# Stanford-ILIAD/PantheonRL

Hardware: AMD Instinct MI355X
Metric: env-steps/sec (all agents) Overcooked-simple PPO self-play (higher is better)
Workload: dtype f32; 1 GPU; OvercookedMultiEnv-v0 layout=simple, PPO self-play (two independent PPO learners per GPU), synthetic (n_envs, n_steps, obs_dim) rollouts; n_envs=1024, n_steps=128, obs_dim=62, features=62, n_logits=6, batch_size=32768, n_epochs=10, agents_per_gpu=2, parallelism=2 agent(s) per gpu x1 gpu(s) = 2 learners (single process), launch_mode=graph, gemm_mode=2, action_masks=none, rollout=scripted, rollout_requested=scripted

## Files before the change

include/pantheon_hip.h:

```cpp
#ifndef PANTHEON_HIP_H
#define PANTHEON_HIP_H

#ifdef __cplusplus
extern "C" {
#endif

#define PH_ABI_VERSION 7
#define PH_HIDDEN 64
#define PH_MAX_COMP 256
#define PH_MAX_LOGITS 64
#define PH_MAX_BOX_ACT 16
#define PH_NSTAT 8
#define PH_MOD_MAX 8
#define PH_MAX_RANKS 16

#define PH_SPACE_BOX 0
#define PH_SPACE_DISCRETE 1

typedef struct ph_ctx ph_ctx;

typedef struct ph_space {
  int kind;
  int n;
  int nvec[PH_MAX_COMP];
// ... 426 lines not shown
                               float *stats_out, const ph_adap_loss *adap );
int ph_adapmult_train(ph_ctx *ctx, const ph_spec *spec, int context_size, const ph_opt_state *opt, const ph_rollout *rb,
                      const ph_ppo_hyper *hyper , int n_epochs, int batch_size, const int *perms,
                      unsigned long long perm_seed, float *stats, const ph_adap_loss *adap );

int ph_bench_ppo_grad(ph_ctx *ctx, const ph_spec *spec, const float *params, const ph_rollout *rb,
                      const ph_ppo_hyper *hyper , int batch_size, int reps, int gemm_mode,
                      float *avg_ms_out );
int ph_bench_gae(ph_ctx *ctx, const ph_rollout *rb, const float *last_values, const float *dones, double gamma,
                 double gae_lambda, int mode, int reps, float *avg_ms_out );

enum {
  PH_BENCH_WEIGHT_IMAGE = 0,
  PH_BENCH_OBS_PLANES = 1,
  PH_BENCH_ADV_STATS = 2,
  PH_BENCH_REDUCE = 3,
  PH_BENCH_REDUCE_WIDE = 4,
  PH_BENCH_ADAM = 5,
  PH_BENCH_STEP_FUSED = 6,
  PH_BENCH_BUFFER_ADD = 7,
  PH_BENCH_SLAB_FLOATS = 8,
  PH_BENCH_NKERN = 9
};
int ph_bench_train_kernels(ph_ctx *ctx, const ph_spec *spec, const ph_opt_state *scratch_opt, const ph_rollout *rb,
                           const ph_ppo_hyper *hyper , int n_epochs, int batch_size, int reps, int gemm_mode,
                           float *us_out );

int ph_feistel_indices(int n, unsigned long long perm_seed, int epoch, int start, int count, int *out );

typedef struct ph_modular {
  int num_partners;
  int n_modules;
  int module_of[PH_MOD_MAX];
  int nomain;
} ph_modular;
int ph_modular_layout(const ph_spec *spec , const ph_modular *mod , ph_layout *main_out ,
                      ph_layout *module_out , int *p_total_out );
int ph_modular_forward(ph_ctx *ctx, const ph_spec *spec, const ph_modular *mod, const float *params, int partner_idx,
                       const float *obs, int n, const unsigned char *action_mask, const float *uniforms,
                       const float *given_actions, unsigned long long seed, unsigned long long counter, int deterministic,
                       int *actions_i32, float *actions_f32, float *values, float *log_probs, float *entropy,
                       float *logits_main , float *logits_partner ,
                       const ph_rollout *rb, int pos, const float *episode_start_in, const float *pending_reward,
                       int gemm_mode);
int ph_modular_train(ph_ctx *ctx, const ph_spec *spec, const ph_modular *mod, const ph_opt_state *opt,
                     int *mod_first ,
// ... 86 lines not shown
```

pantheonrl_amd/_native.py:

```python
from __future__ import annotations

import ctypes as C
import os
from typing import Optional, Sequence

PH_HIDDEN = 64
PH_MAX_COMP = 256
PH_MAX_LOGITS = 64
PH_MAX_BOX_ACT = 16
PH_NSTAT = 8
PH_SPACE_BOX = 0
PH_SPACE_DISCRETE = 1
STAT_NAMES = ("policy_loss", "value_loss", "entropy_loss", "clip_fraction", "approx_kl", "loss", "grad_norm", "applied")

_HERE = os.path.dirname(os.path.abspath(__file__))
LIB_PATH = os.environ.get("PANTHEON_HIP_LIB") or os.path.join(_HERE, "csrc", "libpantheon_hip.so")


class NativeError(RuntimeError):
    """Raised for any non-zero status from the C ABI (message from ph_last_error)."""


class PhSpace(C.Structure):
    _fields_ = [("kind", C.c_int), ("n", C.c_int), ("nvec", C.c_int * PH_MAX_COMP)]
# ... 190 lines not shown
                ("obs_ego", C.c_void_p), ("obs_alt", C.c_void_p), ("episodes", C.c_void_p),
                ("obs_next", C.c_void_p), ("rew1", C.c_void_p), ("rew2", C.c_void_p), ("es_alt", C.c_void_p),
                ("done1", C.c_void_p), ("done2", C.c_void_p), ("running", C.c_void_p), ("can", C.c_void_p),
                ("alt_opens", C.c_void_p), ("ego_opens", C.c_void_p), ("done", C.c_void_p)]

SIGNATURES = {
    "ph_abi_version": [],
    "ph_roundrobin_env_step": [_vp, _vp, _vp, _vp, _vp, _vp, _vp, _vp, _i, _i, C.c_float, _i],
    "ph_last_error": [],
    "ph_device_count": [C.POINTER(_i)],
    "ph_ctx_create": [_i, C.POINTER(_vp)],
    "ph_ctx_destroy": [_vp],
    "ph_ctx_set_stream": [_vp, _vp],
    "ph_ctx_sync": [_vp],
    "ph_graph_begin": [_vp],
    "ph_graph_end": [_vp, C.POINTER(_i)],
    "ph_graph_launch": [_vp, _i],
    "ph_ctx_set_rng_epoch": [_vp, _vp],
    "ph_rng_epoch_advance": [_vp],
    "ph_debug_set_profile_buffer": [_vp, _vp],
    "ph_set_exclusive_device": [_vp, _i],
    "ph_ctx_step_errors": [_vp, C.POINTER(C.c_uint)],
    "ph_debug_weight_image_mismatches": [_vp, C.POINTER(PhSpec), _vp, C.POINTER(C.c_int)],
    "ph_timer_start": [_vp],
    "ph_timer_stop": [_vp, C.POINTER(C.c_float)],
    "ph_layout_of": [C.POINTER(PhSpec), C.POINTER(PhLayout)],
    "ph_debug_split_tables": [C.POINTER(PhSpec), C.POINTER(C.c_int), C.POINTER(C.c_int), C.POINTER(C.c_int)],
    "ph_debug_split_oh_tables": [C.POINTER(PhSpec), _vp, _vp, C.POINTER(_i), C.POINTER(_i), C.POINTER(_i)],
    "ph_buffer_add": [_vp, C.POINTER(PhSpec), C.POINTER(PhRollout), _i, _vp, _vp, _vp, _vp, _vp],
    "ph_buffer_add_reward": [_vp, C.POINTER(PhRollout), _i, _vp, _vp],
    "ph_buffer_add_reward_joint": [_vp, C.POINTER(PhRollout), _i, _vp, _vp, _i, _i, _vp, C.c_float],
    "ph_buffer_reset": [_vp, C.POINTER(PhSpec), C.POINTER(PhRollout)],
    "ph_gae": [_vp, C.POINTER(PhRollout), _vp, _vp, _d, _d, _i],
    "ph_policy_forward": [_vp, C.POINTER(PhSpec), _vp, _vp, _i, _vp, _vp, _vp, _ull, _ull, _i, _vp, _vp, _vp, _vp, _vp,
                          _vp, C.POINTER(PhRollout), _i, _vp, _vp, _i],
    "ph_ctx_set_joint_reward_rule": [_vp, _i],
    "ph_adapmult_layout_of": [C.POINTER(PhSpec), _i, _vp],
    "ph_adapmult_forward": [_vp, C.POINTER(PhSpec), _i, _vp, _vp, _i, _vp, _vp, _vp, _ull, _ull, _i, _vp, _vp, _vp, _vp, _vp,
                            _vp, C.POINTER(PhRollout), _i, _vp],
    "ph_adapmult_minibatch_grad": [_vp, C.POINTER(PhSpec), _i, _vp, C.POINTER(PhRollout), C.POINTER(PhPpoHyper), _vp, _i, _vp, _vp,
                                   _vp],
    "ph_adapmult_train": [_vp, C.POINTER(PhSpec), _i, C.POINTER(PhOptState), C.POINTER(PhRollout), C.POINTER(PhPpoHyper), _i, _i,
                          _vp, _ull, _vp, _vp],
    "ph_policy_act_host": [_vp, C.POINTER(PhSpec), _vp, _vp, _i, _vp, _ull, _ull, _i, _vp, _vp, _vp, C.POINTER(PhRollout), _i, _i],
    "ph_buffer_add_reward_const": [_vp, C.POINTER(PhRollout), _i, C.c_float],
    "ph_policy_step_multi": [_vp, _i, C.POINTER(PhStepCall)],
# ... 245 lines not shown
```

pantheonrl_amd/csrc/ph_abi.hip:

```cpp
#include <dlfcn.h>
#include <hip/hip_runtime.h>
#include <rccl/rccl.h>

#include <atomic>
#include <chrono>
#include <cmath>
#include <cstdio>
#include <cstdint>
#include <cstring>
#include <mutex>
#include <string>
#include <vector>

#include "ph_launch.h"
#include "ph_block.h"
#include "ph_arch.h"
#include "ph_pool.h"

namespace ph {

namespace {
struct LdsGrant {
  const void* kernel;
  int device;
// ... 81 lines not shown
  size_t slabs_cap = 0;
  float* statpart = nullptr;
  size_t statpart_cap = 0;
  float* grad = nullptr;
  size_t grad_cap = 0;
  float* blocksq = nullptr;
  size_t blocksq_cap = 0;
  float* advstats = nullptr;
  size_t advstats_cap = 0;
  float* act_stage_host = nullptr;
  float* act_stage_dev = nullptr;
  size_t act_stage_cap = 0;
  unsigned int* act_done_host = nullptr;
  unsigned int* act_done_dev = nullptr;
  unsigned int act_seq = 0;
  unsigned int* fwd_host_done = nullptr;
  int joint_reward_rule = 0;
  int wimage_zeroed_for = 0;
  size_t wimage_cap = 0;
  bool exclusive = false;
  unsigned short* wimage = nullptr;
  double* advpart = nullptr;
  size_t advpart_cap = 0;
  int* perm_idx = nullptr;
  size_t perm_idx_cap = 0;
  int* perm_phys = nullptr;
  size_t perm_phys_cap = 0;
  uint4* ximg = nullptr;
  size_t ximg_cap = 0;
  uint4* rec_pi = nullptr;
  uint4* rec_vf = nullptr;
  size_t rec_cap = 0;
  uint4* rowrec = nullptr;
  size_t rowrec_cap = 0;
  unsigned long long* step_words = nullptr;
  size_t step_words_cap = 0;
  unsigned int* step_gen = nullptr;
  float* am_buf = nullptr;
  size_t am_buf_cap = 0;
  float* adap_extra = nullptr;
  size_t adap_extra_cap = 0;
  float* adap_loss = nullptr;
  size_t adap_loss_cap = 0;
  float* scalars = nullptr;
  int* stop_flag = nullptr;
  std::vector<SpecCache> specs;
// ... 245 lines not shown
    a.prev_rew = rb->rewards + (row - rb->E);
    a.pending_reward = pending_reward;
  }
  return 0;
}

ph::AdvStatArgs adv_args_epochs(const ph_ctx* ctx, const ph_rollout* rb, const int* perms, unsigned long long perm_seed, int batch,
                                int n_mb) {
  const int N = rb->T * rb->E;
  ph::AdvStatArgs aa{};
  aa.rb_adv = rb->advantages;
  aa.T = rb->T;
  aa.E = rb->E;
  aa.perms = perms;
  aa.perm_n = (uint32_t)N;
  aa.perm_hb = ph::feistel_half_bits((uint32_t)N);
  aa.perm_seed = perm_seed;
  aa.epoch = ctx->rng_epoch;
  aa.N = N;
  aa.batch = batch;
  aa.n_mb = n_mb;
  aa.out = ctx->advstats;
  aa.partial = ctx->advpart;
  aa.idx_out = perms ? nullptr : ctx->perm_idx;
  aa.phys_out = ctx->perm_phys;
  return aa;
}
ph::AdvStatArgs adv_args_minibatch(const ph_ctx* ctx, const ph_rollout* rb, const int* indices, int nb) {
  ph::AdvStatArgs aa{};
  aa.rb_adv = rb->advantages;
  aa.T = rb->T;
  aa.E = rb->E;
  aa.perms = indices;
  aa.perm_hb = 1;
  aa.N = nb;
  aa.batch = nb;
  aa.n_mb = 1;
  aa.out = ctx->advstats;
  aa.partial = ctx->advpart;
  aa.phys_out = ctx->perm_phys;
  return aa;
}

struct MbWalk {
  int ep, start, nb;
  const int* idx;
};
MbWalk minibatch_walk(const ph_ctx* ctx, const int* perms, int N, int n_mb, int batch_size, int mbi) {
  MbWalk w;
  w.ep = mbi / n_mb;
  w.start = (mbi - w.ep * n_mb) * batch_size;
  w.nb = N - w.start < batch_size ? N - w.start : batch_size;
  w.idx = (perms ? perms : ctx->perm_idx) + (size_t)w.ep * N + w.start;
  return w;
}

ph::ReduceArgs reduce_args(const ph_ctx* ctx, const ph_ppo_hyper* hp, const ph_opt_state* opt, int P, int slab_len, const int* map,
                           int nslab, int nb, float* grad, float* stats_out) {
  ph::ReduceArgs r;
  r.slabs = ctx->slabs;
  r.nslab = nslab;
  r.nstatpart = 2 * nslab;
// ... 116 lines not shown
    return fail("hipMalloc(ctx scalars) failed");
  }
  (void)hipMemset(c->scalars, 0, 4 * sizeof(float));
  (void)hipMemset(c->stop_flag, 0, sizeof(int));
  (void)hipEventCreate(&c->ev0);
  (void)hipEventCreate(&c->ev1);
  *out = c;
  return 0;
}

int ph_ctx_destroy(ph_ctx* ctx) {
  DevGuard dev_guard(ctx);
  if (!ctx) return 0;
  (void)hipStreamSynchronize(ctx->stream);
  for (auto g : ctx->graphs)
    if (g) (void)hipGraphExecDestroy(g);
  for (auto& s : ctx->specs) {
    if (s.obs_off) (void)hipFree(s.obs_off);
    if (s.slab_map) (void)hipFree(s.slab_map);
    if (s.slab_map_split) (void)hipFree(s.slab_map_split);
    if (s.wimage_map) (void)hipFree(s.wimage_map);
    if (s.act_off) (void)hipFree(s.act_off);
  }
  void* ptrs[] = {ctx->wimage, ctx->mw.act, ctx->mw.maps, ctx->mw.kl_sum, ctx->mw.scratch, ctx->advpart, ctx->p2p_dev, ctx->slabs, ctx->statpart, ctx->grad, ctx->blocksq, ctx->advstats, ctx->perm_idx, ctx->perm_phys, ctx->ximg, ctx->rec_pi, ctx->rec_vf, ctx->rowrec, ctx->step_words, ctx->step_gen, ctx->scalars, ctx->stop_flag,
                  ctx->adap_extra, ctx->adap_loss, ctx->am_buf, ctx->pool_dev, ctx->pool_order, ctx->pool_tiles};
  for (void* p : ptrs)
    if (p) (void)hipFree(p);
  if (ctx->act_stage_host) (void)hipHostFree(ctx->act_stage_host);
  if (ctx->act_done_host) (void)hipHostFree(ctx->act_done_host);
  if (ctx->ev0) (void)hipEventDestroy(ctx->ev0);
  if (ctx->ev1) (void)hipEventDestroy(ctx->ev1);
  if (ctx->ev_grad) (void)hipEventDestroy(ctx->ev_grad);
  (void)ph_comm_destroy(ctx);
  delete ctx;
  return 0;
}

int ph_ctx_set_joint_reward_rule(ph_ctx* ctx, int rule) {
  if (!ctx) return fail("null ctx");
  if (rule != PH_JOINT_MATCH_BONUS && rule != PH_JOINT_RPS) return fail("ph_ctx_set_joint_reward_rule: unknown rule");
  ctx->joint_reward_rule = rule;
  return 0;
}

int ph_ctx_set_stream(ph_ctx* ctx, void* hip_stream) {
  DevGuard dev_guard(ctx);
  if (!ctx) return fail("null ctx");
// ... 1443 lines not shown
  }
  PH_HIP(ph::launch_obs_planes(rb->observations, (int)rows, nd.D, nd.F, ph::grad_fast_fold(nd) ? 1 : 0, ctx->ximg, rb->advantages,
                               rb->log_probs, rb->actions, rb->returns, rb->values, ctx->rowrec, ctx->stream));
  return 0;
}
void fill_adv_records(ph::AdvStatArgs& aa, const ph_ctx* ctx, const ph::NetDims& nd, const ph_rollout* rb) {
  aa.rec_pi_out = nd.split == 1 ? ctx->rec_pi : nullptr;
  aa.rec_vf_out = nd.split == 1 ? ctx->rec_vf : nullptr;
  aa.rowrec = (nd.split == 1 && rb->advantages && rb->log_probs && rb->actions && rb->returns && rb->values) ? ctx->rowrec : nullptr;
  aa.rb_logp = rb->log_probs;
  aa.rb_act = rb->actions;
  aa.rb_ret = rb->returns;
  aa.rb_val = rb->values;
}


void select_gemm(ph::NetDims& nd, int gemm_mode) {
  nd.split = (gemm_mode == 2 && nd.slab_map_split != nullptr) ? nd.split_kind : 0;
  if (nd.split) nd.slab_map = nd.slab_map_split;
}

int slab_len_of(const ph::NetDims& nd) { return nd.split ? nd.slab_len_split : (nd.slab_map ? 2 * ph::RS_NET : nd.lay.P); }

int ensure_train_ws(ph_ctx* ctx, int P, int slab_len, int nwg_max, int n_mb_total, size_t n_idx = 0, size_t n_phys = 0) {
  if (n_phys && ensure(ctx, ctx->perm_phys, ctx->perm_phys_cap, n_phys)) return 1;
  if (ensure(ctx, ctx->slabs, ctx->slabs_cap, (size_t)nwg_max * slab_len)) return 1;
  if (ensure(ctx, ctx->statpart, ctx->statpart_cap, (size_t)2 * nwg_max * ph::NSTATP)) return 1;
  if (ensure(ctx, ctx->grad, ctx->grad_cap, (size_t)P)) return 1;
  if (ensure(ctx, ctx->blocksq, ctx->blocksq_cap, (size_t)ph::reduce_blocks(slab_len))) return 1;
  if (ensure(ctx, ctx->advstats, ctx->advstats_cap, (size_t)n_mb_total * 2)) return 1;
  if (ensure(ctx, ctx->advpart, ctx->advpart_cap, (size_t)n_mb_total * 2 * ph::ADV_SPLIT)) return 1;
  if (n_idx && ensure(ctx, ctx->perm_idx, ctx->perm_idx_cap, n_idx)) return 1;
  const size_t n_words = (size_t)ph::reduce_blocks(slab_len) + 1;
  if (n_words > ctx->step_words_cap) {
    if (ensure(ctx, ctx->step_words, ctx->step_words_cap, n_words)) return 1;
    PH_HIP(hipMemsetAsync(ctx->step_words, 0, n_words * sizeof(unsigned long long), ctx->stream));
  }
  if (!ctx->step_gen) {
    if (ctx->capturing) return fail("workspace would grow inside graph capture: run the same call once outside capture first");
    PH_HIP(hipMalloc((void**)&ctx->step_gen, 4 * sizeof(unsigned int)));
    PH_HIP(hipMemsetAsync(ctx->step_gen, 0, 4 * sizeof(unsigned int), ctx->stream));
  }
  return 0;
}

bool step_fused_wanted(const ph_ctx* ctx, int slab_len, bool alone) {
  return alone && ctx->exclusive && ctx->step_words && ctx->step_gen &&
         ph::step_fused_fits(ph::reduce_blocks(slab_len), slab_len, ctx->num_cu);
}

}

namespace {

// ... 643 lines not shown
  auto launch = [&](int i) {
    const MbWalk w = minibatch_walk(ctx, nullptr, N, n_mb, nb, i % n_mb);
    g.idx = w.idx;
    g.idx_phys = ctx->perm_phys + w.start;
    g.mb_start = w.start;
    g.rec_pi = ctx->rec_pi ? ctx->rec_pi + w.start : nullptr;
    g.rec_vf = ctx->rec_vf ? ctx->rec_vf + w.start : nullptr;
    g.advstats = ctx->advstats + 2 * (size_t)(i % n_mb);
    return hip_rc(ph::launch_ppo_grad(g, pl.nwg, gemm_mode, s), "ph_bench_ppo_grad: launch_ppo_grad");
  };
  return time_reps(ctx, n_mb, reps, launch, avg_ms_out);
}

int ph_bench_gae(ph_ctx* ctx, const ph_rollout* rb, const float* last_values, const float* dones, double gamma,
                 double gae_lambda, int mode, int reps, float* avg_ms_out) {
  DevGuard dev_guard(ctx);
  if (!ctx || !last_values || !dones || !avg_ms_out) return fail("ph_bench_gae: null argument");
  if (check_rb(rb)) return 1;
  if (reps <= 0 || mode < 0 || mode > 2) return fail("ph_bench_gae: bad arguments");
  return time_reps(ctx, 1, reps, [&](int) {
    return hip_rc(ph::launch_gae(rb->rewards, rb->values, rb->episode_starts, last_values, dones, rb->advantages, rb->returns,
                                 rb->T, rb->E, gamma, gae_lambda, mode, ctx->stream), "ph_bench_gae: launch_gae");
  }, avg_ms_out);
}

int ph_bench_train_kernels(ph_ctx* ctx, const ph_spec* spec, const ph_opt_state* opt, const ph_rollout* rb,
                           const ph_ppo_hyper* hp, int n_epochs, int batch_size, int reps, int gemm_mode, float* us_out) {
  DevGuard dev_guard(ctx);
  if (!us_out) return fail("ph_bench_train_kernels: null argument");
  if (reps <= 0) return fail("ph_bench_train_kernels: reps must be positive");
  for (int i = 0; i < PH_BENCH_NKERN; ++i) us_out[i] = 0.f;
  TrainPlan t;
  if (train_prepare("ph_bench_train_kernels", t, ctx, spec, opt, rb, hp, n_epochs, batch_size, nullptr, 12345ull, nullptr, gemm_mode))
    return 1;
  hipStream_t s = ctx->stream;
  auto timed = [&](int slot, auto&& fn) -> int {
    float ms = 0.f;
    if (time_reps(ctx, 1, reps, [&](int) { return fn(); }, &ms)) return 1;
    us_out[slot] = 1e3f * ms;
    return 0;
  };
  auto hip = [](hipError_t e) { return hip_rc(e, "ph_bench_train_kernels"); };
  if (t.nd.split) {
    if (timed(PH_BENCH_WEIGHT_IMAGE, [&] { return rebuild_weight_image(ctx, t.nd, opt->params); })) return 1;
    if (timed(PH_BENCH_OBS_PLANES, [&] { return build_grad_pack(ctx, t.nd, rb, (size_t)n_epochs * t.N); })) return 1;
  }
// ... 562 lines not shown
```

pantheonrl_amd/csrc/ph_launch.h:

```cpp
#pragma once
#include "ph_device.h"

namespace ph {

__host__ __device__ inline unsigned p2p_stamp32(unsigned long long epoch, int T, int t) {
  return (unsigned)(epoch * (unsigned long long)T + (unsigned long long)t + 1ull);
}

__device__ __forceinline__ void p2p_note_timeout(unsigned long long* error, int kind, int t, unsigned long long index,
                                                 unsigned long long want, unsigned long long seen) {
  if (atomicAdd(error, 1ull) == 0ull) {
    error[1] = (unsigned long long)(unsigned)kind | ((unsigned long long)(unsigned)(t & 0xffffff) << 8) | (index << 32);
    error[2] = want;
    error[3] = seen;
  }
}

__device__ __forceinline__ void poll_backoff(int& polls) {
  if (polls < 16) __builtin_amdgcn_s_sleep(2);
  else if (polls < 64) __builtin_amdgcn_s_sleep(16);
  else __builtin_amdgcn_s_sleep(127);
  ++polls;
}

// ... 136 lines not shown
  }
  return env_major_to_phys(n, a.T, a.E);
}

constexpr int ADV_SPLIT = 32;
constexpr int ADV_THREADS = 256;
struct AdvStatArgs {
  const float* rb_adv;
  int T, E;
  const int* perms;
  uint32_t perm_n, perm_hb;
  uint64_t perm_seed;
  const unsigned long long* epoch;
  int N, batch, n_mb;
  float* out;
  double* partial;
  int* idx_out;
  int* phys_out;
  uint4* rec_pi_out = nullptr;
  uint4* rec_vf_out = nullptr;
  const float *rb_logp = nullptr, *rb_act = nullptr, *rb_ret = nullptr, *rb_val = nullptr;
  const uint4* rowrec = nullptr;
  int* clear_flag = nullptr;
};

struct ReduceArgs {
  const float* slabs;
  int nslab, P;
  int slab_len;
  const int* map;
  float* grad;
  float* blocksq;
  const float* statpart;
  int nstatpart;
  float* stats_out;
  int nb;
  float ent_coef, vf_coef, target_kl;
  int* stop_flag;
  int* step;
  float* scalars;
  const float* extra = nullptr;
  int n_extra = 0, extra_len = 0, extra_cut = 0, extra_lo = 0, extra_hi = 0;
  const float* extra_loss = nullptr;
  float extra_norm = 0.f;
  float extra_coef = 0.f;
  float* extra_loss_out = nullptr;
// ... 308 lines not shown
```

pantheonrl_amd/csrc/ph_ppo.hip:

```cpp
#include "ph_launch.h"
#include "ph_split.h"
#include "ph_step.h"

namespace ph {


template <int N>
__device__ __forceinline__ float lds_colsum(const float* p, int stride, float s) {
#pragma unroll
  for (int r0 = 0; r0 < N; r0 += 16) {
    float t[16];
#pragma unroll
    for (int i = 0; i < 16; ++i) t[i] = p[(r0 + i) * stride];
    __builtin_amdgcn_sched_barrier(0);
#pragma unroll
    for (int i = 0; i < 16; ++i) s += t[i];
  }
  return s;
}
template <int N>
__device__ __forceinline__ float lds_coldot(const float* p, int stride, const float* q, int qstride, float s) {
#pragma unroll
  for (int r0 = 0; r0 < N; r0 += 16) {
    float t[16], u[16];
// ... 730 lines not shown

void grad_plan(const NetDims& nd, int nb, int num_cu, int* ntiles, int* nwg) {
  *ntiles = (nb + 63) / 64;
  *nwg = *ntiles < num_cu ? *ntiles : num_cu;
  if (nd.split == 2 && *nwg > num_cu / 2 && num_cu >= 2) *nwg = num_cu / 2;
}

hipError_t launch_ppo_grad(const GradArgs& a, int nwg, int gemm_mode, hipStream_t s) {
  if (a.nd.split == 2) return launch_ppo_grad_split_oh(a, nwg, s);
  if (a.nd.split) return launch_ppo_grad_split(a, nwg, s);
  if (grad_fast_eligible(a.nd)) return launch_ppo_grad_fast(a, nwg, gemm_mode, s);
  if (a.nd.Lp != 32 && a.nd.Lp != 64) return hipErrorInvalidValue;
  const bool lp64 = a.nd.Lp == 64;
  if (gemm_mode == 1) return lp64 ? launch_grad_shape<64, true>(a, nwg, s) : launch_grad_shape<32, true>(a, nwg, s);
  return lp64 ? launch_grad_shape<64, false>(a, nwg, s) : launch_grad_shape<32, false>(a, nwg, s);
}

__device__ __forceinline__ void st_rec(uint4* p, const uint4& v) {
  typedef unsigned int u32x4_t __attribute__((ext_vector_type(4)));
  __builtin_nontemporal_store((u32x4_t){v.x, v.y, v.z, v.w}, reinterpret_cast<u32x4_t*>(p));
}
__global__ __launch_bounds__(ADV_THREADS) void adv_stats_kernel(AdvStatArgs a) {
  __shared__ double sh[2][ADV_THREADS / 64];
  const int mb = blockIdx.x / ADV_SPLIT, seg = blockIdx.x - mb * ADV_SPLIT;
  const int ep = mb / a.n_mb, k = mb - ep * a.n_mb;
  const int start = k * a.batch;
  const int nb = (a.N - start < a.batch) ? a.N - start : a.batch;
  const uint64_t key = epoch_key(a.perm_seed + (a.epoch ? *a.epoch : 0ull), ep);
  const int tid = threadIdx.x, lane = tid & 63, wave = tid >> 6;
  if (a.clear_flag && blockIdx.x == 0 && tid == 0) *a.clear_flag = 0;
  const int chunk = (nb + ADV_SPLIT - 1) / ADV_SPLIT;
  const int lo = seg * chunk, hi = (lo + chunk < nb) ? lo + chunk : nb;
  auto value = [&](int i) -> double {
    if (i >= hi) return 0.0;
    int n;
    if (a.perms) {
      n = a.perms[(size_t)ep * a.N + start + i];
    } else {
      n = (int)feistel_perm((uint32_t)(start + i), a.perm_n, a.perm_hb, key);
      if (a.idx_out) a.idx_out[(size_t)ep * a.N + start + i] = n;
    }
    const int phys = env_major_to_phys(n, a.T, a.E);
    if (a.phys_out) a.phys_out[(size_t)ep * a.N + start + i] = phys;
    float adv;
    if (a.rec_pi_out && a.rowrec) {
      const uint4 rp = a.rowrec[2 * (size_t)phys], rv = a.rowrec[2 * (size_t)phys + 1];
// ... 12 lines not shown
    return (double)adv;
  };
  double s = 0.0, q = 0.0;
  for (int i = lo + tid; i < hi; i += 4 * ADV_THREADS) {
    const double v0 = value(i), v1 = value(i + ADV_THREADS), v2 = value(i + 2 * ADV_THREADS), v3 = value(i + 3 * ADV_THREADS);
    s += (v0 + v1) + (v2 + v3);
    q += (v0 * v0 + v1 * v1) + (v2 * v2 + v3 * v3);
  }
  for (int off = 32; off > 0; off >>= 1) {
    s += __shfl_down(s, off, 64);
    q += __shfl_down(q, off, 64);
  }
  if (lane == 0) {
    sh[0][wave] = s;
    sh[1][wave] = q;
  }
  __syncthreads();
  if (tid == 0) {
    double ts = 0.0, tq = 0.0;
    for (int w = 0; w < ADV_THREADS / 64; ++w) {
      ts += sh[0][w];
      tq += sh[1][w];
    }
    a.partial[((size_t)mb * ADV_SPLIT + seg) * 2 + 0] = ts;
    a.partial[((size_t)mb * ADV_SPLIT + seg) * 2 + 1] = tq;
  }
}
__global__ void adv_finalize_kernel(AdvStatArgs a, int n_total) {
  const int mb = blockIdx.x * blockDim.x + threadIdx.x;
  if (mb >= n_total) return;
  const int k = mb % a.n_mb;
  const int start = k * a.batch;
  const int nb = (a.N - start < a.batch) ? a.N - start : a.batch;
  double ts = 0.0, tq = 0.0;
  for (int seg = 0; seg < ADV_SPLIT; ++seg) {
    ts += a.partial[((size_t)mb * ADV_SPLIT + seg) * 2 + 0];
    tq += a.partial[((size_t)mb * ADV_SPLIT + seg) * 2 + 1];
  }
  const double mean = ts / (double)nb;
  double var = (nb > 1) ? (tq - (double)nb * mean * mean) / (double)(nb - 1) : 0.0;
  if (var < 0.0) var = 0.0;
  a.out[2 * mb + 0] = (float)mean;
  a.out[2 * mb + 1] = (float)sqrt(var);
}
hipError_t launch_adv_stats(const AdvStatArgs& a, int n_total, hipStream_t s) {
  hipLaunchKernelGGL(adv_stats_kernel, dim3(n_total * ADV_SPLIT), dim3(ADV_THREADS), 0, s, a);
  hipLaunchKernelGGL(adv_finalize_kernel, dim3((n_total + 63) / 64), dim3(64), 0, s, a, n_total);
  return hipGetLastError();
}

constexpr int OP_ROWS = 32;
struct RowScalars {
  const float *adv, *logp, *act, *ret, *val;
  uint4* rowrec;
};
__global__ __launch_bounds__(256) void obs_planes_kernel(const float* __restrict__ obs, int n, int D, int F, int fold,
                                                         uint4* __restrict__ image, RowScalars rs) {
  __shared__ float xs[OP_ROWS][65];
  const int tid = threadIdx.x;
  const size_t row0 = (size_t)blockIdx.x * OP_ROWS;
  const int nrow = (row0 + OP_ROWS <= (size_t)n) ? OP_ROWS : (int)((size_t)n > row0 ? (size_t)n - row0 : 0);
  const float* src = obs + row0 * D;
  for (int e = tid; e < nrow * D; e += 256) {
    const int r = e / D, f = e - r * D;
    if (f < F) xs[r][f] = __builtin_nontemporal_load(src + e);
  }
  __syncthreads();
  const int r = tid >> 3, g = tid & 7;
  const size_t row = row0 + r;
  if (row > (size_t)n) return;
// ... 7 lines not shown
  bf8 pl[3];
#pragma unroll
  for (int e = 0; e < 8; ++e) {
    const int f = 8 * g + e;
    float x = 0.f;
    if (row < (size_t)n) x = f < F ? xs[r][f] : ((fold && f == HID - 1) ? 1.f : 0.f);
    __bf16 h, m, l;
    split1(x, h, m, l);
    pl[0][e] = h;
    pl[1][e] = m;
    pl[2][e] = l;
  }
#pragma unroll
  for (int p = 0; p < 3; ++p) image[row * XIMG_ROW_U4 + p * 8 + g] = __builtin_bit_cast(uint4, pl[p]);
}
hipError_t launch_obs_planes(const float* obs, int n, int D, int F, int fold, uint4* image, const float* adv, const float* logp,
                             const float* act, const float* ret, const float* val, uint4* rowrec, hipStream_t s) {
  const size_t blocks = ((size_t)n + 1 + OP_ROWS - 1) / OP_ROWS;
  RowScalars rs{adv, logp, act, ret, val, (adv && logp && act && ret && val) ? rowrec : nullptr};
  hipLaunchKernelGGL(obs_planes_kernel, dim3((unsigned)blocks), dim3(256), 0, s, obs, n, D, F, fold, image, rs);
  return hipGetLastError();
}

template <int VEC>
__global__ __launch_bounds__(RED_PARAMS * 4) void ppo_reduce_kernel(ReduceArgs a) {
  __shared__ float lds_union[4 * RED_PARAMS];
  static_assert(4 * RED_PARAMS >= 32 * NSTATP + NSTATP || 4 * RED_PARAMS >= 32 * NSTATP, "statistics scratch within the slab scratch");
  float (*gsum)[RED_PARAMS] = reinterpret_cast<float (*)[RED_PARAMS]>(lds_union);
  float (*part)[NSTATP] = reinterpret_cast<float (*)[NSTATP]>(lds_union);
  __shared__ float means[NSTATP];
  const int tid = threadIdx.x;
  if (*a.stop_flag != 0) {
    if (blockIdx.x == 0 && tid < PH_NSTAT && a.stats_out) a.stats_out[tid] = 0.f;
    if (blockIdx.x == 0 && tid == 0) {
      a.scalars[1] = 0.f;
      a.scalars[2] = 0.f;
    }
    return;
  }
  if (blockIdx.x == gridDim.x - 1) {
    (void)reduce_statistics(a, part, means, true);
    return;
  }
  const int dst = reduce_dst(a, blockIdx.x);
  const float g = reduce_positions<VEC>(a, gsum, dst, blockIdx.x);
  if (tid < 64) {
    if (dst >= 0) a.grad[dst] = g;
    float q = g * g;
    for (int off = 32; off > 0; off >>= 1) q += __shfl_down(q, off, 64);
    if (tid == 0) a.blocksq[blockIdx.x] = q;
  }
}

template <int VEC>
__global__ __launch_bounds__(RED_PARAMS * 4) void ppo_step_kernel(StepArgs s) {
  __shared__ float gsum[4][RED_PARAMS];
  __shared__ float part[32][NSTATP];
  __shared__ float means[NSTATP];
  const int nblk = gridDim.x - 1;
  const int stopped = *s.r.stop_flag;
  const unsigned tag = *s.gen + 1u;
  const int step_new = *s.ad.step + 1;
  const unsigned err = *s.sweep_error;
  step_body<VEC>(s, blockIdx.x, nblk, tag, step_new, gsum, part, means, nullptr, stopped, err);
}

int reduce_blocks(int slab_len) { return (slab_len + RED_PARAMS - 1) / RED_PARAMS; }
static int reduce_vec(int slab_len, int exclusive) { return (slab_len % 4 == 0 && exclusive) ? 4 : (slab_len % 2 == 0 ? 2 : 1); }
bool step_fused_fits(int nblk, int slab_len, int num_cu) {
  if (nblk + 1 > 64 * 16) return false;
  static int per_cu[3] = {-1, -1, -1};
  const int vec = reduce_vec(slab_len, 1);
  int& v = per_cu[vec == 4 ? 2 : vec - 1];
  if (v < 0) {
    int api = 0;
    const void* fn = vec == 4 ? (const void*)ppo_step_kernel<4> : vec == 2 ? (const void*)ppo_step_kernel<2> : (const void*)ppo_step_kernel<1>;
    hipError_t e = hipOccupancyMaxActiveBlocksPerMultiprocessor(&api, fn, RED_PARAMS * 4, 0);
    v = (e == hipSuccess && api > 1) ? api - 1 : 0;
  }
  return (long long)v * num_cu >= (long long)nblk + 1;
}
hipError_t launch_ppo_step(const ReduceArgs& r, const AdamArgs& ad, unsigned long long* words, unsigned int* gen,
                           unsigned int* sweep_error, unsigned long long timeout, hipStream_t st) {
  StepArgs s;
  s.r = r;
  s.ad = ad;
  s.words = words;
  s.gen = gen;
  s.timeout = timeout;
  s.sweep_error = sweep_error;
  const int nblk = reduce_blocks(r.slab_len);
  if ((unsigned long long)r.nslab * (unsigned long long)r.slab_len * sizeof(float) >= (1ull << 32)) return hipErrorInvalidValue;
  switch (reduce_vec(r.slab_len, 1)) {
    case 4: hipLaunchKernelGGL(ppo_step_kernel<4>, dim3(nblk + 1), dim3(RED_PARAMS * 4), 0, st, s); break;
    case 2: hipLaunchKernelGGL(ppo_step_kernel<2>, dim3(nblk + 1), dim3(RED_PARAMS * 4), 0, st, s); break;
    default: hipLaunchKernelGGL(ppo_step_kernel<1>, dim3(nblk + 1), dim3(RED_PARAMS * 4), 0, st, s); break;
  }
  return hipGetLastError();
}
hipError_t launch_ppo_reduce(const ReduceArgs& a, hipStream_t s) {
  const dim3 grid(reduce_blocks(a.slab_len) + 1), block(RED_PARAMS * 4);
  if ((unsigned long long)a.nslab * (unsigned long long)a.slab_len * sizeof(float) >= (1ull << 32)) return hipErrorInvalidValue;
  switch (reduce_vec(a.slab_len, a.wide)) {
    case 4: hipLaunchKernelGGL(ppo_reduce_kernel<4>, grid, block, 0, s, a); break;
    case 2: hipLaunchKernelGGL(ppo_reduce_kernel<2>, grid, block, 0, s, a); break;
    default: hipLaunchKernelGGL(ppo_reduce_kernel<1>, grid, block, 0, s, a); break;
  }
  return hipGetLastError();
}

__global__ __launch_bounds__(256) void ppo_adam_kernel(AdamArgs a) {
  __shared__ float sh[4];
  __shared__ AdamScalars ks;
  const int tid = threadIdx.x;
  const int p = blockIdx.x * blockDim.x + tid;
  const bool live = p < a.P;
  float gr = 0.f, m0 = 0.f, v0 = 0.f, p0 = 0.f;
  int i0 = -1, i1 = -1;
  if (live) {
    gr = a.grad[p];
    m0 = a.m[p];
    v0 = a.v[p];
    p0 = a.params[p];
    if (a.wimage) {
      i0 = a.wimage_map[2 * p];
      i1 = a.wimage_map[2 * p + 1];
// ... 84 lines not shown
```

pantheonrl_amd/csrc/ph_step.h:

```cpp
#pragma once
#include "ph_launch.h"
#include "ph_split.h"

namespace ph {

constexpr int RED_PARAMS = 64, RED_SUB = 16, RED_SHIFT = 6;

struct AdamScalars {
  float coef, ss, bc2s;
};
__device__ __forceinline__ AdamScalars adam_scalars(float total_norm, float max_norm, int step, float lr, float beta1, float beta2) {
  AdamScalars k;
  const float cc = max_norm / (total_norm + 1e-6f);
  k.coef = cc < 1.0f ? cc : 1.0f;
  const double t = (double)step;
  const double bc1 = 1.0 - pow((double)beta1, t);
  const double bc2 = 1.0 - pow((double)beta2, t);
  k.ss = (float)((double)lr / bc1);
  k.bc2s = (float)sqrt(bc2);
  return k;
}
__device__ __forceinline__ float adam_apply(float grad, const AdamScalars& k, float beta1, float beta2, float eps, float m0, float v0,
                                            float p0, float* m_out, float* v_out) {
#pragma clang fp contract(off)
// ... 12 lines not shown
                                             float* v_p, float* param_p) {
  float m, v;
  const float pn = adam_apply(grad, k, beta1, beta2, eps, *m_p, *v_p, *param_p, &m, &v);
  *m_p = m;
  *v_p = v;
  *param_p = pn;
  return pn;
}
template <int VEC>
struct RedVec;
template <>
struct RedVec<1> { using T = float; };
template <>
struct RedVec<2> { using T = float2; };
template <>
struct RedVec<4> { using T = float4; };
__device__ __forceinline__ int reduce_dst(const ReduceArgs& a, int blk) {
  const int tid = threadIdx.x;
  if (tid >= RED_PARAMS) return -1;
  const int p = blk * RED_PARAMS + tid;
  return p < a.slab_len ? (a.map ? a.map[p] : p) : -1;
}
template <int VEC, bool COH, typename RSRC>
__device__ __forceinline__ void range_walk(const ReduceArgs& a, const RSRC& rsrc, unsigned stride, int per, bool full, int k0, int p0,
                                           float (&range)[VEC]) {
  using VT = typename RedVec<VEC>::T;
  const int n = (k0 + per <= a.nslab ? per : a.nslab - k0);
  float acc[8][VEC];
#pragma unroll
  for (int u = 0; u < 8; ++u)
#pragma unroll
    for (int c = 0; c < VEC; ++c) acc[u][c] = 0.f;
  if (p0 < a.slab_len) {
    const unsigned lane_off = (unsigned)k0 * stride + (unsigned)p0 * (unsigned)sizeof(float);
    constexpr int AUX = COH ? 16 : 0;
    auto ld = [&](int j) -> VT {
      if constexpr (VEC == 4) return __builtin_bit_cast(VT, __builtin_amdgcn_raw_buffer_load_b128(rsrc, lane_off, (unsigned)j * stride, AUX));
      else if constexpr (VEC == 2) return __builtin_bit_cast(VT, __builtin_amdgcn_raw_buffer_load_b64(rsrc, lane_off, (unsigned)j * stride, AUX));
      else return __builtin_bit_cast(VT, __builtin_amdgcn_raw_buffer_load_b32(rsrc, lane_off, (unsigned)j * stride, AUX));
    };
    auto add = [&](float (&dst)[VEC], const VT& x) {
      const float* xv = reinterpret_cast<const float*>(&x);
#pragma unroll
      for (int c = 0; c < VEC; ++c) dst[c] += xv[c];
    };
    int j = 0;
    if (full) {
      for (; j + 15 < per; j += 16) {
        VT x0[8], x1[8];
// ... 17 lines not shown
      }
#pragma unroll
      for (int u = 0; u < 8; ++u) add(acc[u], x0[u]);
    }
  }
#pragma unroll
  for (int c = 0; c < VEC; ++c)
    range[c] = ((acc[0][c] + acc[1][c]) + (acc[2][c] + acc[3][c])) + ((acc[4][c] + acc[5][c]) + (acc[6][c] + acc[7][c]));
}
__device__ __forceinline__ float extra_terms(const ReduceArgs& a, int dst, float g) {
  if (a.n_extra <= 0) return g;
  const int e = dst < a.extra_cut ? dst : ((dst >= a.extra_lo && dst < a.extra_hi) ? a.extra_cut + (dst - a.extra_lo) : -1);
  if (e < 0) return g;
  for (int k0 = 0; k0 < a.n_extra; k0 += 8) {
    float x[8];
#pragma unroll
    for (int u = 0; u < 8; ++u) x[u] = (k0 + u < a.n_extra) ? a.extra[(size_t)(k0 + u) * a.extra_len + e] : 0.f;
#pragma unroll
    for (int u = 0; u < 8; ++u)
      if (k0 + u < a.n_extra) g += x[u];
  }
  return g;
}
template <int VEC, bool COH = false>
__device__ __forceinline__ float reduce_positions(const ReduceArgs& a, float (*gsum)[RED_PARAMS], int dst, int blk) {
  static_assert(VEC == 1 || VEC == 2 || VEC == 4, "positions per lane");
  constexpr int LP = RED_PARAMS / VEC;
  constexpr int TURNS = 4 / VEC;
  const int tid = threadIdx.x, lane = tid & 63;
  const int wave = __builtin_amdgcn_readfirstlane(tid >> RED_SHIFT);
  const int lp = lane % LP, gw = lane / LP;
  const int p0 = blk * RED_PARAMS + lp * VEC;
  const int per = (a.nslab + RED_SUB - 1) / RED_SUB;
  const bool full = per * RED_SUB == a.nslab;
  const unsigned stride = (unsigned)a.slab_len * (unsigned)sizeof(float);
  const auto rsrc = __builtin_amdgcn_make_buffer_rsrc(const_cast<float*>(a.slabs), 0, (int)((unsigned)a.nslab * stride), 0x00020000);
  float rs[TURNS][VEC];
#pragma unroll
  for (int t = 0; t < TURNS; ++t)
#pragma unroll
    for (int c = 0; c < VEC; ++c) rs[t][c] = 0.f;
#pragma unroll 1
  for (int turn = 0; turn < TURNS; ++turn) {
    const int sub = wave * 4 + gw * TURNS + turn;
    float range[VEC];
    range_walk<VEC, COH>(a, rsrc, stride, per, full, sub * per, p0, range);
#pragma unroll
    for (int c = 0; c < VEC; ++c) {
#pragma unroll
      for (int t = 0; t < TURNS; ++t) rs[t][c] = (turn == t) ? range[c] : rs[t][c];
    }
  }
  {
    float q[VEC];
#pragma unroll
    for (int c = 0; c < VEC; ++c) q[c] = rs[0][c];
#pragma unroll
    for (int g = 0; g < VEC; ++g)
#pragma unroll
      for (int turn = 0; turn < TURNS; ++turn) {
        if (g == 0 && turn == 0) continue;
#pragma unroll
        for (int c = 0; c < VEC; ++c) q[c] += (g == 0) ? rs[turn][c] : __shfl(rs[turn][c], lp + g * LP, 64);
      }
    if (gw == 0) {
#pragma unroll
      for (int c = 0; c < VEC; ++c) gsum[wave][lp * VEC + c] = q[c];
    }
  }
// ... 205 lines not shown
```

Baseline: 117.3 million agent-steps/s.

## Fuse advantage-stat finalize into stats kernel via tickets; add lean vec4 reduce path

Removes the separate adv_finalize kernel launch: each segment block writes its partial sums atomically, bumps a per-minibatch ticket, and the last arriving block computes the mean and std and resets the ticket. Also changes reduce_vec so VEC=4 is chosen whenever the slab length allows, not only in exclusive mode. The non-wide VEC=4 reduce now walks slabs in two halves with four accumulators to cut register pressure, and the wide path gets its own kernel. Risks include ticket memory-ordering correctness and a different summation order.

```diff
diff --git a/include/pantheon_hip.h b/include/pantheon_hip.h
--- a/include/pantheon_hip.h
+++ b/include/pantheon_hip.h
@@ -472,6 +472,10 @@
   PH_BENCH_SLAB_FLOATS = 8,
   PH_BENCH_NKERN = 9
 };
+int ph_debug_reduce_slabs(ph_ctx *ctx, const float *slabs, int nslab, int slab_len, int wide, int stop, float *grad_out,
+                          float *blocksq_out);
+int ph_debug_adv_stats(ph_ctx *ctx, const ph_rollout *rb, const int *perms, int n_epochs, int batch_size, float *stats_out,
+                       void *rec_pi_out, void *rec_vf_out);
 int ph_bench_train_kernels(ph_ctx *ctx, const ph_spec *spec, const ph_opt_state *scratch_opt, const ph_rollout *rb,
                            const ph_ppo_hyper *hyper , int n_epochs, int batch_size, int reps, int gemm_mode,
                            float *us_out );
diff --git a/pantheonrl_amd/_native.py b/pantheonrl_amd/_native.py
--- a/pantheonrl_amd/_native.py
+++ b/pantheonrl_amd/_native.py
@@ -236,6 +236,8 @@
     "ph_set_exclusive_device": [_vp, _i],
     "ph_ctx_step_errors": [_vp, C.POINTER(C.c_uint)],
     "ph_debug_weight_image_mismatches": [_vp, C.POINTER(PhSpec), _vp, C.POINTER(C.c_int)],
+    "ph_debug_reduce_slabs": [_vp, _vp, _i, _i, _i, _i, _vp, _vp],
+    "ph_debug_adv_stats": [_vp, C.POINTER(PhRollout), _vp, _i, _i, _vp, _vp, _vp],
     "ph_timer_start": [_vp],
     "ph_timer_stop": [_vp, C.POINTER(C.c_float)],
     "ph_layout_of": [C.POINTER(PhSpec), C.POINTER(PhLayout)],
diff --git a/pantheonrl_amd/csrc/ph_abi.hip b/pantheonrl_amd/csrc/ph_abi.hip
--- a/pantheonrl_amd/csrc/ph_abi.hip
+++ b/pantheonrl_amd/csrc/ph_abi.hip
@@ -127,6 +127,8 @@
   unsigned short* wimage = nullptr;
   double* advpart = nullptr;
   size_t advpart_cap = 0;
+  unsigned int* advticket = nullptr;
+  size_t advticket_cap = 0;
   int* perm_idx = nullptr;
   size_t perm_idx_cap = 0;
   int* perm_phys = nullptr;
@@ -418,6 +420,7 @@
   aa.n_mb = n_mb;
   aa.out = ctx->advstats;
   aa.partial = ctx->advpart;
+  aa.ticket = ctx->advticket;
   aa.idx_out = perms ? nullptr : ctx->perm_idx;
   aa.phys_out = ctx->perm_phys;
   return aa;
@@ -434,6 +437,7 @@
   aa.n_mb = 1;
   aa.out = ctx->advstats;
   aa.partial = ctx->advpart;
+  aa.ticket = ctx->advticket;
   aa.phys_out = ctx->perm_phys;
   return aa;
 }
@@ -596,7 +600,7 @@
     if (s.wimage_map) (void)hipFree(s.wimage_map);
     if (s.act_off) (void)hipFree(s.act_off);
   }
-  void* ptrs[] = {ctx->wimage, ctx->mw.act, ctx->mw.maps, ctx->mw.kl_sum, ctx->mw.scratch, ctx->advpart, ctx->p2p_dev, ctx->slabs, ctx->statpart, ctx->grad, ctx->blocksq, ctx->advstats, ctx->perm_idx, ctx->perm_phys, ctx->ximg, ctx->rec_pi, ctx->rec_vf, ctx->rowrec, ctx->step_words, ctx->step_gen, ctx->scalars, ctx->stop_flag,
+  void* ptrs[] = {ctx->wimage, ctx->mw.act, ctx->mw.maps, ctx->mw.kl_sum, ctx->mw.scratch, ctx->advpart, ctx->advticket, ctx->p2p_dev, ctx->slabs, ctx->statpart, ctx->grad, ctx->blocksq, ctx->advstats, ctx->perm_idx, ctx->perm_phys, ctx->ximg, ctx->rec_pi, ctx->rec_vf, ctx->rowrec, ctx->step_words, ctx->step_gen, ctx->scalars, ctx->stop_flag,
                   ctx->adap_extra, ctx->adap_loss, ctx->am_buf, ctx->pool_dev, ctx->pool_order, ctx->pool_tiles};
   for (void* p : ptrs)
     if (p) (void)hipFree(p);
@@ -2086,14 +2090,22 @@
 
 int slab_len_of(const ph::NetDims& nd) { return nd.split ? nd.slab_len_split : (nd.slab_map ? 2 * ph::RS_NET : nd.lay.P); }
 
+int ensure_adv_ws(ph_ctx* ctx, int n_mb_total) {
+  if (ensure(ctx, ctx->advstats, ctx->advstats_cap, (size_t)n_mb_total * 2)) return 1;
+  if (ensure(ctx, ctx->advpart, ctx->advpart_cap, (size_t)n_mb_total * 2 * ph::ADV_SPLIT)) return 1;
+  if ((size_t)n_mb_total > ctx->advticket_cap) {
+    if (ensure(ctx, ctx->advticket, ctx->advticket_cap, (size_t)n_mb_total)) return 1;
+    PH_HIP(hipMemsetAsync(ctx->advticket, 0, (size_t)n_mb_total * sizeof(unsigned int), ctx->stream));
+  }
+  return 0;
+}
 int ensure_train_ws(ph_ctx* ctx, int P, int slab_len, int nwg_max, int n_mb_total, size_t n_idx = 0, size_t n_phys = 0) {
   if (n_phys && ensure(ctx, ctx->perm_phys, ctx->perm_phys_cap, n_phys)) return 1;
   if (ensure(ctx, ctx->slabs, ctx->slabs_cap, (size_t)nwg_max * slab_len)) return 1;
   if (ensure(ctx, ctx->statpart, ctx->statpart_cap, (size_t)2 * nwg_max * ph::NSTATP)) return 1;
   if (ensure(ctx, ctx->grad, ctx->grad_cap, (size_t)P)) return 1;
   if (ensure(ctx, ctx->blocksq, ctx->blocksq_cap, (size_t)ph::reduce_blocks(slab_len))) return 1;
-  if (ensure(ctx, ctx->advstats, ctx->advstats_cap, (size_t)n_mb_total * 2)) return 1;
-  if (ensure(ctx, ctx->advpart, ctx->advpart_cap, (size_t)n_mb_total * 2 * ph::ADV_SPLIT)) return 1;
+  if (ensure_adv_ws(ctx, n_mb_total)) return 1;
   if (n_idx && ensure(ctx, ctx->perm_idx, ctx->perm_idx_cap, n_idx)) return 1;
   const size_t n_words = (size_t)ph::reduce_blocks(slab_len) + 1;
   if (n_words > ctx->step_words_cap) {
@@ -2783,6 +2795,62 @@
     return hip_rc(ph::launch_gae(rb->rewards, rb->values, rb->episode_starts, last_values, dones, rb->advantages, rb->returns,
                                  rb->T, rb->E, gamma, gae_lambda, mode, ctx->stream), "ph_bench_gae: launch_gae");
   }, avg_ms_out);
+}
+
+int ph_debug_reduce_slabs(ph_ctx* ctx, const float* slabs, int nslab, int slab_len, int wide, int stop, float* grad_out,
+                          float* blocksq_out) {
+  DevGuard dev_guard(ctx);
+  if (!ctx || !slabs || !grad_out || !blocksq_out) return fail("ph_debug_reduce_slabs: null argument");
+  if (nslab <= 0 || slab_len <= 0) return fail("ph_debug_reduce_slabs: empty slabs");
+  hipStream_t s = ctx->stream;
+  ph::ReduceArgs r;
+  r.slabs = slabs;
+  r.nslab = nslab;
+  r.P = slab_len;
+  r.slab_len = slab_len;
+  r.map = nullptr;
+  r.grad = grad_out;
+  r.blocksq = blocksq_out;
+  r.statpart = nullptr;
+  r.nstatpart = 0;
+  r.stats_out = nullptr;
+  r.nb = 1;
+  r.ent_coef = r.vf_coef = 0.f;
+  r.target_kl = -1.f;
+  r.stop_flag = ctx->stop_flag;
+  r.step = nullptr;
+  r.scalars = ctx->scalars;
+  r.wide = wide ? 1 : 0;
+  PH_HIP(ph::launch_set_int(ctx->stop_flag, stop ? 1 : 0, s));
+  PH_HIP(ph::launch_ppo_reduce(r, s));
+  PH_HIP(ph::launch_set_int(ctx->stop_flag, 0, s));
+  PH_HIP(hipStreamSynchronize(s));
+  return 0;
+}
+
+int ph_debug_adv_stats(ph_ctx* ctx, const ph_rollout* rb, const int* perms, int n_epochs, int batch_size, float* stats_out,
+                       void* rec_pi_out, void* rec_vf_out) {
+  DevGuard dev_guard(ctx);
+  if (!ctx || !rb || !perms || !stats_out) return fail("ph_debug_adv_stats: null argument");
+  const int N = rb->T * rb->E;
+  if (N <= 0 || n_epochs <= 0 || batch_size <= 0) return fail("ph_debug_adv_stats: empty call");
+  if ((rec_pi_out || rec_vf_out) && !(rec_pi_out && rec_vf_out && rb->log_probs && rb->actions && rb->returns && rb->values))
+    return fail("ph_debug_adv_stats: the records need both outputs and the buffer's scalar arrays");
+  const int n_mb = (N + batch_size - 1) / batch_size;
+  if (ensure_adv_ws(ctx, n_epochs * n_mb)) return 1;
+  hipStream_t s = ctx->stream;
+  ph::AdvStatArgs aa = adv_args_epochs(ctx, rb, perms, 0ull, batch_size, n_mb);
+  aa.phys_out = nullptr;
+  aa.rec_pi_out = static_cast<uint4*>(rec_pi_out);
+  aa.rec_vf_out = static_cast<uint4*>(rec_vf_out);
+  aa.rb_logp = rb->log_probs;
+  aa.rb_act = rb->actions;
+  aa.rb_ret = rb->returns;
+  aa.rb_val = rb->values;
+  PH_HIP(ph::launch_adv_stats(aa, n_epochs * n_mb, s));
+  PH_HIP(hipMemcpyAsync(stats_out, ctx->advstats, (size_t)n_epochs * n_mb * 2 * sizeof(float), hipMemcpyDeviceToHost, s));
+  PH_HIP(hipStreamSynchronize(s));
+  return 0;
 }
 
 int ph_bench_train_kernels(ph_ctx* ctx, const ph_spec* spec, const ph_opt_state* opt, const ph_rollout* rb,
diff --git a/pantheonrl_amd/csrc/ph_launch.h b/pantheonrl_amd/csrc/ph_launch.h
--- a/pantheonrl_amd/csrc/ph_launch.h
+++ b/pantheonrl_amd/csrc/ph_launch.h
@@ -182,6 +182,7 @@
   const float *rb_logp = nullptr, *rb_act = nullptr, *rb_ret = nullptr, *rb_val = nullptr;
   const uint4* rowrec = nullptr;
   int* clear_flag = nullptr;
+  unsigned int* ticket = nullptr;
 };
 
 struct ReduceArgs {
diff --git a/pantheonrl_amd/csrc/ph_ppo.hip b/pantheonrl_amd/csrc/ph_ppo.hip
--- a/pantheonrl_amd/csrc/ph_ppo.hip
+++ b/pantheonrl_amd/csrc/ph_ppo.hip
@@ -776,6 +776,8 @@
 }
 __global__ __launch_bounds__(ADV_THREADS) void adv_stats_kernel(AdvStatArgs a) {
   __shared__ double sh[2][ADV_THREADS / 64];
+  __shared__ double fin[2 * ADV_SPLIT];
+  __shared__ int last_arrived;
   const int mb = blockIdx.x / ADV_SPLIT, seg = blockIdx.x - mb * ADV_SPLIT;
   const int ep = mb / a.n_mb, k = mb - ep * a.n_mb;
   const int start = k * a.batch;
@@ -834,30 +836,36 @@
       ts += sh[0][w];
       tq += sh[1][w];
     }
-    a.partial[((size_t)mb * ADV_SPLIT + seg) * 2 + 0] = ts;
-    a.partial[((size_t)mb * ADV_SPLIT + seg) * 2 + 1] = tq;
-  }
-}
-__global__ void adv_finalize_kernel(AdvStatArgs a, int n_total) {
-  const int mb = blockIdx.x * blockDim.x + threadIdx.x;
-  if (mb >= n_total) return;
-  const int k = mb % a.n_mb;
-  const int start = k * a.batch;
-  const int nb = (a.N - start < a.batch) ? a.N - start : a.batch;
-  double ts = 0.0, tq = 0.0;
-  for (int seg = 0; seg < ADV_SPLIT; ++seg) {
-    ts += a.partial[((size_t)mb * ADV_SPLIT + seg) * 2 + 0];
-    tq += a.partial[((size_t)mb * ADV_SPLIT + seg) * 2 + 1];
-  }
-  const double mean = ts / (double)nb;
-  double var = (nb > 1) ? (tq - (double)nb * mean * mean) / (double)(nb - 1) : 0.0;
-  if (var < 0.0) var = 0.0;
-  a.out[2 * mb + 0] = (float)mean;
-  a.out[2 * mb + 1] = (float)sqrt(var);
+    double* part = a.partial + ((size_t)mb * ADV_SPLIT + seg) * 2;
+    __hip_atomic_store(part + 0, ts, __ATOMIC_RELAXED, __HIP_MEMORY_SCOPE_AGENT);
+    __hip_atomic_store(part + 1, tq, __ATOMIC_RELAXED, __HIP_MEMORY_SCOPE_AGENT);
+    __builtin_amdgcn_fence(__ATOMIC_RELEASE, "workgroup");
+    __builtin_amdgcn_s_waitcnt(0x0F70);
+    const bool last = __hip_atomic_fetch_add(a.ticket + mb, 1u, __ATOMIC_RELAXED, __HIP_MEMORY_SCOPE_AGENT) == (unsigned)(ADV_SPLIT - 1);
+    last_arrived = last ? 1 : 0;
+  }
+  __syncthreads();
+  if (!last_arrived) return;
+  if (tid < 2 * ADV_SPLIT)
+    fin[tid] = __hip_atomic_load(a.partial + (size_t)mb * ADV_SPLIT * 2 + tid, __ATOMIC_RELAXED, __HIP_MEMORY_SCOPE_AGENT);
+  __syncthreads();
+  if (tid == 0) {
+    double ts = 0.0, tq = 0.0;
+    for (int s2 = 0; s2 < ADV_SPLIT; ++s2) {
+      ts += fin[2 * s2 + 0];
+      tq += fin[2 * s2 + 1];
+    }
+    const double mean = ts / (double)nb;
+    double var = (nb > 1) ? (tq - (double)nb * mean * mean) / (double)(nb - 1) : 0.0;
+    if (var < 0.0) var = 0.0;
+    a.out[2 * mb + 0] = (float)mean;
+    a.out[2 * mb + 1] = (float)sqrt(var);
+    a.ticket[mb] = 0u;
+  }
 }
 hipError_t launch_adv_stats(const AdvStatArgs& a, int n_total, hipStream_t s) {
+  if (!a.ticket) return hipErrorInvalidValue;
   hipLaunchKernelGGL(adv_stats_kernel, dim3(n_total * ADV_SPLIT), dim3(ADV_THREADS), 0, s, a);
-  hipLaunchKernelGGL(adv_finalize_kernel, dim3((n_total + 63) / 64), dim3(64), 0, s, a, n_total);
   return hipGetLastError();
 }
 
@@ -911,13 +919,13 @@
   return hipGetLastError();
 }
 
-template <int VEC>
-__global__ __launch_bounds__(RED_PARAMS * 4) void ppo_reduce_kernel(ReduceArgs a) {
+template <int VEC, bool LEAN>
+__device__ __forceinline__ void reduce_kernel_body(const ReduceArgs& a) {
   __shared__ float lds_union[4 * RED_PARAMS];
-  static_assert(4 * RED_PARAMS >= 32 * NSTATP + NSTATP || 4 * RED_PARAMS >= 32 * NSTATP, "statistics scratch within the slab scratch");
+  static_assert(4 * RED_PARAMS >= 32 * NSTATP, "statistics scratch within the slab scratch");
   float (*gsum)[RED_PARAMS] = reinterpret_cast<float (*)[RED_PARAMS]>(lds_union);
   float (*part)[NSTATP] = reinterpret_cast<float (*)[NSTATP]>(lds_union);
-  __shared__ float means[NSTATP];
+  float* means = lds_union;
   const int tid = threadIdx.x;
   if (*a.stop_flag != 0) {
     if (blockIdx.x == 0 && tid < PH_NSTAT && a.stats_out) a.stats_out[tid] = 0.f;
@@ -932,7 +940,7 @@
     return;
   }
   const int dst = reduce_dst(a, blockIdx.x);
-  const float g = reduce_positions<VEC>(a, gsum, dst, blockIdx.x);
+  const float g = reduce_positions<VEC, false, LEAN>(a, gsum, dst, blockIdx.x);
   if (tid < 64) {
     if (dst >= 0) a.grad[dst] = g;
     float q = g * g;
@@ -940,6 +948,11 @@
     if (tid == 0) a.blocksq[blockIdx.x] = q;
   }
 }
+template <int VEC>
+__global__ __launch_bounds__(RED_PARAMS * 4) void ppo_reduce_kernel(ReduceArgs a) {
+  reduce_kernel_body<VEC, VEC == 4>(a);
+}
+__global__ __launch_bounds__(RED_PARAMS * 4) void ppo_reduce_wide_kernel(ReduceArgs a) { reduce_kernel_body<4, false>(a); }
 
 template <int VEC>
 __global__ __launch_bounds__(RED_PARAMS * 4) void ppo_step_kernel(StepArgs s) {
@@ -955,11 +968,11 @@
 }
 
 int reduce_blocks(int slab_len) { return (slab_len + RED_PARAMS - 1) / RED_PARAMS; }
-static int reduce_vec(int slab_len, int exclusive) { return (slab_len % 4 == 0 && exclusive) ? 4 : (slab_len % 2 == 0 ? 2 : 1); }
+static int reduce_vec(int slab_len) { return slab_len % 4 == 0 ? 4 : (slab_len % 2 == 0 ? 2 : 1); }
 bool step_fused_fits(int nblk, int slab_len, int num_cu) {
   if (nblk + 1 > 64 * 16) return false;
   static int per_cu[3] = {-1, -1, -1};
-  const int vec = reduce_vec(slab_len, 1);
+  const int vec = reduce_vec(slab_len);
   int& v = per_cu[vec == 4 ? 2 : vec - 1];
   if (v < 0) {
     int api = 0;
@@ -980,7 +993,7 @@
   s.sweep_error = sweep_error;
   const int nblk = reduce_blocks(r.slab_len);
   if ((unsigned long long)r.nslab * (unsigned long long)r.slab_len * sizeof(float) >= (1ull << 32)) return hipErrorInvalidValue;
-  switch (reduce_vec(r.slab_len, 1)) {
+  switch (reduce_vec(r.slab_len)) {
     case 4: hipLaunchKernelGGL(ppo_step_kernel<4>, dim3(nblk + 1), dim3(RED_PARAMS * 4), 0, st, s); break;
     case 2: hipLaunchKernelGGL(ppo_step_kernel<2>, dim3(nblk + 1), dim3(RED_PARAMS * 4), 0, st, s); break;
     default: hipLaunchKernelGGL(ppo_step_kernel<1>, dim3(nblk + 1), dim3(RED_PARAMS * 4), 0, st, s); break;
@@ -990,7 +1003,14 @@
 hipError_t launch_ppo_reduce(const ReduceArgs& a, hipStream_t s) {
   const dim3 grid(reduce_blocks(a.slab_len) + 1), block(RED_PARAMS * 4);
   if ((unsigned long long)a.nslab * (unsigned long long)a.slab_len * sizeof(float) >= (1ull << 32)) return hipErrorInvalidValue;
-  switch (reduce_vec(a.slab_len, a.wide)) {
+  if (a.slab_len % 4 == 0 && a.wide) {
+    hipLaunchKernelGGL(ppo_reduce_wide_kernel, grid, block, 0, s, a);
+    return hipGetLastError();
+  }
+#ifdef PH_AB_REDUCE_VEC2
+  if (a.slab_len % 2 == 0) { hipLaunchKernelGGL(ppo_reduce_kernel<2>, grid, block, 0, s, a); return hipGetLastError(); }
+#endif
+  switch (reduce_vec(a.slab_len)) {
     case 4: hipLaunchKernelGGL(ppo_reduce_kernel<4>, grid, block, 0, s, a); break;
     case 2: hipLaunchKernelGGL(ppo_reduce_kernel<2>, grid, block, 0, s, a); break;
     default: hipLaunchKernelGGL(ppo_reduce_kernel<1>, grid, block, 0, s, a); break;
diff --git a/pantheonrl_amd/csrc/ph_step.h b/pantheonrl_amd/csrc/ph_step.h
--- a/pantheonrl_amd/csrc/ph_step.h
+++ b/pantheonrl_amd/csrc/ph_step.h
@@ -58,9 +58,76 @@
   return p < a.slab_len ? (a.map ? a.map[p] : p) : -1;
 }
 template <int VEC, bool COH, typename RSRC>
+__device__ __forceinline__ void range_walk_halves(const ReduceArgs& a, const RSRC& rsrc, unsigned stride, int per, bool full, int k0,
+                                                  int p0, float (&range)[VEC]) {
+  using VT = typename RedVec<VEC>::T;
+  const int n = (k0 + per <= a.nslab ? per : a.nslab - k0);
+  float half_sum[2][VEC] = {};
+#pragma unroll 1
+  for (int h = 0; h < 2; ++h) {
+    float acc[4][VEC];
+#pragma unroll
+    for (int u = 0; u < 4; ++u)
+#pragma unroll
+      for (int c = 0; c < VEC; ++c) acc[u][c] = 0.f;
+    if (p0 < a.slab_len) {
+      const unsigned lane_off = (unsigned)k0 * stride + (unsigned)p0 * (unsigned)sizeof(float);
+      constexpr int AUX = COH ? 16 : 0;
+      auto ld = [&](int j) -> VT {
+        if constexpr (VEC == 4) return __builtin_bit_cast(VT, __builtin_amdgcn_raw_buffer_load_b128(rsrc, lane_off, (unsigned)j * stride, AUX));
+        else if constexpr (VEC == 2) return __builtin_bit_cast(VT, __builtin_amdgcn_raw_buffer_load_b64(rsrc, lane_off, (unsigned)j * stride, AUX));
+        else return __builtin_bit_cast(VT, __builtin_amdgcn_raw_buffer_load_b32(rsrc, lane_off, (unsigned)j * stride, AUX));
+      };
+      auto add = [&](float (&dst)[VEC], const VT& x) {
+        const float* xv = reinterpret_cast<const float*>(&x);
+#pragma unroll
+        for (int c = 0; c < VEC; ++c) dst[c] += xv[c];
+      };
+      const int j4 = 4 * h;
+      int j = 0;
+      if (full) {
+        for (; j + 15 < per; j += 16) {
+          VT x0[4], x1[4];
+#pragma unroll
+          for (int u = 0; u < 4; ++u) x0[u] = ld(j + j4 + u);
+#pragma unroll
+          for (int u = 0; u < 4; ++u) x1[u] = ld(j + 8 + j4 + u);
+          __builtin_amdgcn_sched_barrier(0);
+#pragma unroll
+          for (int u = 0; u < 4; ++u) add(acc[u], x0[u]);
+#pragma unroll
+          for (int u = 0; u < 4; ++u) add(acc[u], x1[u]);
+        }
+      }
+      for (; j < per; j += 8) {
+        VT x0[4];
+#pragma unroll
+        for (int u = 0; u < 4; ++u) {
+          x0[u] = VT{};
+          if (j + j4 + u < n) x0[u] = ld(j + j4 + u);
+        }
+#pragma unroll
+        for (int u = 0; u < 4; ++u) add(acc[u], x0[u]);
+      }
+    }
+#pragma unroll
+    for (int c = 0; c < VEC; ++c) {
+      const float f = (acc[0][c] + acc[1][c]) + (acc[2][c] + acc[3][c]);
+      half_sum[0][c] = h == 0 ? f : half_sum[0][c];
+      half_sum[1][c] = f;
+    }
+  }
+#pragma unroll
+  for (int c = 0; c < VEC; ++c) range[c] = half_sum[0][c] + half_sum[1][c];
+}
+template <int VEC, bool COH, bool LEAN = false, typename RSRC>
 __device__ __forceinline__ void range_walk(const ReduceArgs& a, const RSRC& rsrc, unsigned stride, int per, bool full, int k0, int p0,
                                            float (&range)[VEC]) {
   using VT = typename RedVec<VEC>::T;
+  if constexpr (LEAN) {
+    range_walk_halves<VEC, COH>(a, rsrc, stride, per, full, k0, p0, range);
+    return;
+  }
   const int n = (k0 + per <= a.nslab ? per : a.nslab - k0);
   float acc[8][VEC];
 #pragma unroll
@@ -124,7 +191,7 @@
   }
   return g;
 }
-template <int VEC, bool COH = false>
+template <int VEC, bool COH = false, bool LEAN = false>
 __device__ __forceinline__ float reduce_positions(const ReduceArgs& a, float (*gsum)[RED_PARAMS], int dst, int blk) {
   static_assert(VEC == 1 || VEC == 2 || VEC == 4, "positions per lane");
   constexpr int LP = RED_PARAMS / VEC;
@@ -146,7 +213,7 @@
   for (int turn = 0; turn < TURNS; ++turn) {
     const int sub = wave * 4 + gw * TURNS + turn;
     float range[VEC];
-    range_walk<VEC, COH>(a, rsrc, stride, per, full, sub * per, p0, range);
+    range_walk<VEC, COH, LEAN>(a, rsrc, stride, per, full, sub * per, p0, range);
 #pragma unroll
     for (int c = 0; c < VEC; ++c) {
 #pragma unroll
```

Result: no change. 118.0 million agent-steps/s (median of 4 runs) (+0.7%).
